# JaneliaSciComp/BigStitcher-Spark

Hardware: NVIDIA H100
Metric: tile-pairs/sec (phase-corr, 512^3 uint16 overlaps) (higher is better)
Workload: dtype f32

## Files before the change

### bigstitcher-spark_b200/csrc/pcm.cu

```cuda
#include <algorithm>
#include <cmath>
#include <cstring>

#include "bs_internal.cuh"
#include "pcm_fft.cuh"

#define PCM_THREADS 256
#define PCM_KMAX 32
#define PCM_SMEM_MAX 232448

extern __shared__ __align__(16) float2 bs_sm[];

struct XR2CArgs {
    const void* img[2];
    float2* spec[2];
    int dtype;
    int dx, dy, dz;
    int Px, Py, Pz, M, pitch;
    int ex;
    int Ex, Ey, Ez;
    const int* idx_x; const float* w_x;
    const int* idx_y; const float* w_y;
    const int* idx_z; const float* w_z;
    const float2* tw;
    FftPlan plan;
    int lshift;
};

__device__ __forceinline__ float load_voxel(const void* p, int dtype, size_t i) {
    if (dtype == BS_DTYPE_U16) return (float)__ldg((const unsigned short*)p + i);
    if (dtype == BS_DTYPE_F32) return __ldg((const float*)p + i);
    return (float)__ldg((const unsigned char*)p + i);
}

#define XR_UNROLL 5
template <class F>
__global__ void __launch_bounds__(PCM_THREADS) k_fft_x_r2c(const __grid_constant__ XR2CArgs a) {
    const int M = F::kStatic ? F::N : a.M;
    const int lshift = F::kStatic ? F::LSHIFT : a.lshift;
    const int LB = 1 << lshift, ls = LB + 1;
    const int Px = 2 * M;
    const int pitch = F::kStatic ? ((F::N + 1 + 15) / 16) * 16 : a.pitch;
    float2* tw = bs_sm;
    float2* b0 = bs_sm + Px;
    float2* b1 = b0 + M * ls;
    const int zp = blockIdx.y, y0 = blockIdx.x * LB, im = blockIdx.z;
    float2* __restrict__ spec = a.spec[im];
    const size_t rowbase = ((size_t)zp * a.Py + y0) * pitch;
    const int nlines = min(LB, a.Py - y0);
    if (zp >= a.Ez || y0 >= a.Ey) {
        const float4 z4 = make_float4(0.f, 0.f, 0.f, 0.f);
        float4* d4 = reinterpret_cast<float4*>(spec + rowbase);
        for (int i = threadIdx.x; i < nlines * (pitch >> 1); i += blockDim.x) d4[i] = z4;
        return;
    }
    for (int i = threadIdx.x; i < Px; i += blockDim.x) tw[i] = a.tw[i];
    const int lane = threadIdx.x & 31, wid = threadIdx.x >> 5;
// ... 107 lines not shown
                 "l"(src), "r"(bytes), "r"(smem_u32(bar))
                 : "memory");
}

struct XR2CTmaArgs {
    XR2CArgs x;
    int n_groups;
    int n_items;
    int row_bytes;
    int esize;
};

template <class F>
__global__ void __launch_bounds__(PCM_THREADS) k_fft_x_r2c_tma(const __grid_constant__ XR2CTmaArgs t) {
    const XR2CArgs& a = t.x;
    const int M = F::kStatic ? F::N : a.M;
    const int lshift = F::kStatic ? F::LSHIFT : a.lshift;
    const int LB = 1 << lshift, ls = LB + 1;
    const int Px = 2 * M;
    const int pitch = F::kStatic ? ((F::N + 1 + 15) / 16) * 16 : a.pitch;
    float2* tw = bs_sm;
    float2* b0 = bs_sm + Px;
    float2* b1 = b0 + M * ls;
    unsigned char* raw = reinterpret_cast<unsigned char*>(b1 + M * ls);
    unsigned long long* bars = reinterpret_cast<unsigned long long*>(raw + 2 * (size_t)LB * t.row_bytes);
    const int lane = threadIdx.x & 31, wid = threadIdx.x >> 5;
    constexpr int NW = PCM_THREADS / 32;

    for (int i = threadIdx.x; i < Px; i += blockDim.x) tw[i] = a.tw[i];
    if (threadIdx.x == 0) {
        mbar_init(&bars[0], 1);
        mbar_init(&bars[1], 1);
        asm volatile("fence.mbarrier_init.release.cluster;" ::: "memory");
    }
    __syncthreads();
// ... 153 lines not shown
        static_assert(UTW + F::Tw::total <= 2 * F::N, "stage tables must fit the twiddle area");
        for (int i = threadIdx.x; i < UTW; i += blockDim.x) tw[i] = a.tw[i];
        F::Tw::build(tw + UTW, a.tw, threadIdx.x, blockDim.x);
    } else {
        for (int i = threadIdx.x; i < Px; i += blockDim.x) tw[i] = a.tw[i];
    }
    if (t.use_tma && lane == 0) {
        mbar_init(&bars[0], 1);
        mbar_init(&bars[1], 1);
        asm volatile("fence.mbarrier_init.release.cluster;" ::: "memory");
    }
    __syncthreads();

    typename F::Tw twr;
    twr.init(F::kSmemTw ? tw + UTW : tw, lane);
    constexpr bool kRegU = F::kStatic && !F::kSmemTw;
    constexpr int UIT = F::kStatic ? (F::N / 2 + 1 + 31) / 32 : 1;
    float2 utw[kRegU ? UIT : 1];
    if constexpr (kRegU) {
#pragma unroll
        for (int i = 0; i < UIT; ++i) utw[i] = tw[min(lane + 32 * i, M)];
    }

    const long long gw = (long long)blockIdx.x * NW + wid, gstride = (long long)gridDim.x * NW;
    const int e0 = a.ex;
    auto src_row = [&](long long line, int& im, int& zp, int& yp) -> long long {
        yp = (int)(line % a.Py);
        const long long r = line / a.Py;
        zp = (int)(r % a.Pz);
        im = (int)(r / a.Pz);
        if (zp >= a.Ez || yp >= a.Ey) return -1;
        return (long long)a.idx_z[zp] * a.dy + a.idx_y[yp];
    };
    auto prefetch = [&](long long line, int buf) {
        int im, zp, yp;
        const long long row = src_row(line, im, zp, yp);
        if (row < 0) return;
// ... 58 lines not shown
        }
        __syncwarp();
        const float2* res = F::run(A, B, tw, twr, a.plan, 2, lane);
        auto untangle = [&](int k, float2 w) {
            const float2 Zk = res[k];
            const float2 Zm = p_mul(res[k == 0 ? 0 : M - k], make_float2(1.f, -1.f));
            const float2 S = caddf(Zk, Zm), Dd = csubf(Zk, Zm);
            const float2 wD = cmulf(w, Dd);
            __stcg(srow + k, cscale(0.5f, cadd_mi(S, wD)));
            if (2 * k != M) __stcg(srow + (M - k), p_mul(cadd_pi(S, wD), make_float2(0.5f, -0.5f)));
        };
        if (F::kStatic) {
#pragma unroll
            for (int i = 0; i < UIT; ++i) {
                const int k = lane + 32 * i;
                if (2 * k <= M) untangle(k, kRegU ? utw[kRegU ? i : 0] : tw[k]);
            }
        } else {
            for (int k = lane; 2 * k <= M; k += 32) untangle(k, tw[k]);
        }
        for (int k = M + 1 + lane; k < pitch; k += 32) __stcg(srow + k, make_float2(0.f, 0.f));
        __syncwarp();
    }
}

#define XW_MAXV 10
template <class F>
__global__ void __launch_bounds__(PCM_THREADS, 3) k_fft_x_c2r_w(const __grid_constant__ XC2RArgs a) {
    const int M = F::kStatic ? F::N : a.M;
    const int Px = 2 * M;
    const int pitch = F::kStatic ? ((F::N + 1 + 15) / 16) * 16 : a.pitch;
    constexpr int NW = PCM_THREADS / 32;
    const int lane = threadIdx.x & 31, wid = threadIdx.x >> 5;
    float2* tw = bs_sm;
    float2* A = bs_sm + Px + (size_t)wid * 2 * (M + 1);
    float2* B = A + (M + 1);
    for (int i = threadIdx.x; i < Px; i += blockDim.x) tw[i] = a.tw[i];
    __syncthreads();
    typename F::Tw twr;
    twr.init(tw, lane);
    constexpr int UIT = F::kStatic ? (F::N / 2 + 1 + 31) / 32 : 1;
    const long long n_lines = (long long)a.Py * a.Pz;
    const long long gw = (long long)blockIdx.x * NW + wid, gstride = (long long)gridDim.x * NW;
    float2 nxt[XW_MAXV];
    auto load_row = [&](long long line) {
        const float2* srow = a.spec + (size_t)line * pitch;
#pragma unroll
        for (int u = 0; u < XW_MAXV; ++u) {
            const int k = lane + 32 * u;
            nxt[u] = (k <= M) ? __ldcg(srow + k) : make_float2(0.f, 0.f);
        }
    };
    if (gw < n_lines) load_row(gw);
    for (long long line = gw; line < n_lines; line += gstride) {
#pragma unroll
        for (int u = 0; u < XW_MAXV; ++u) {
            const int k = lane + 32 * u;
            if (k <= M) B[k] = make_float2(nxt[u].x, -nxt[u].y);
        }
        __syncwarp();
        if (line + gstride < n_lines) load_row(line + gstride);
        auto tangle = [&](int k, float2 wc) {
            const float2 Xk = B[k];
            const float2 Xm = p_mul(B[M - k], make_float2(1.f, -1.f));
            const float2 S = caddf(Xk, Xm), Dd = csubf(Xk, Xm);
            const float2 O = cmulf(Dd, wc);
            A[k] = p_mul(cadd_pi(S, O), make_float2(0.5f, -0.5f));
            if (k != 0 && 2 * k != M) A[M - k] = cscale(0.5f, cadd_mi(S, O));
        };
        if (F::kStatic) {
#pragma unroll
            for (int i = 0; i < UIT; ++i) {
                const int k = lane + 32 * i;
                if (2 * k <= M) tangle(k, p_mul(tw[k], make_float2(1.f, -1.f)));
            }
        } else {
            for (int k = lane; 2 * k <= M; k += 32) tangle(k, p_mul(tw[k], make_float2(1.f, -1.f)));
        }
        __syncwarp();
        const float2* res = F::run(A, B, tw, twr, a.plan, 2, lane);
        float2* row = a.spec + (size_t)line * pitch;
        for (int n = lane; n < M; n += 32) {
            const float2 r = res[n];
            __stcg(row + n, make_float2(r.x * a.scale, -r.y * a.scale));
        }
        __syncwarp();
    }
}

typedef FftWStatic<270, 2, 9, 6, 5> FftW270;
typedef FftWStaticS<270, 2, 9, 6, 5> FftW270S;

struct StridedArgs {
    float2* a;
    float2* b;
    long long estride;
    long long ostride;
    const float2* tw;
    FftPlan plan;
    int tshift;
    int mode;
    float thresh;
};

template <int UNR>
__device__ __forceinline__ void tile_load(float2* dst, const float2* g, long long estride, int N, int tshift) {
// ... 23 lines not shown
    const float4* s4 = reinterpret_cast<const float4*>(src);
#pragma unroll 4
    for (int i = threadIdx.x; i < nvec; i += blockDim.x)
        __stcg(reinterpret_cast<float4*>(g + (long long)(i >> vshift) * estride) + (i & vmask), s4[i]);
}

__device__ __forceinline__ float2 unit_or_zero(float2 x, float thresh) {
    const float m2 = x.x * x.x + x.y * x.y;
    if (m2 < thresh * thresh) return make_float2(0.f, 0.f);
    const float inv = rsqrtf(m2);
    return make_float2(x.x * inv, x.y * inv);
}

template <class F>
__global__ void __launch_bounds__(PCM_THREADS, 3) k_fft_strided(const __grid_constant__ StridedArgs a) {
    const int tshift = F::kStatic ? F::LSHIFT : a.tshift;
    const int TW = 1 << tshift, N = F::kStatic ? F::N : a.plan.n;
    const int twpad = (N + 1) & ~1;
    float2* tw = bs_sm;
    float2* B0 = bs_sm + twpad;
    float2* B1 = B0 + (size_t)N * TW;
    const size_t base = (size_t)blockIdx.y * a.ostride + (size_t)blockIdx.x * TW;
    for (int i = threadIdx.x; i < N; i += blockDim.x) tw[i] = a.tw[i];
    if (a.mode == 0) {
        float2* g = (blockIdx.z ? a.b : a.a) + base;
        tile_load<9>(B0, g, a.estride, N, tshift);
        __syncthreads();
        const float2* res = F::run(B0, B1, tw, a.plan, tshift, TW, 1);
        tile_store(g, res, a.estride, N, tshift);
    } else {
        float2* B2 = B1 + (size_t)N * TW;
        tile_load<9>(B0, a.a + base, a.estride, N, tshift);
// ... 20 lines not shown
}
__device__ __forceinline__ void cp_async_commit() { asm volatile("cp.async.commit_group;" ::: "memory"); }
template <int N>
__device__ __forceinline__ void cp_async_wait() { asm volatile("cp.async.wait_group %0;" ::"n"(N) : "memory"); }

struct StridedPipeArgs {
    StridedArgs s;
    int tiles_x;
    int n_other;
    int n_tiles;
};

template <class F>
__global__ void __launch_bounds__(PCM_THREADS, 2) k_fft_strided_pipe(const __grid_constant__ StridedPipeArgs p) {
    const StridedArgs& a = p.s;
    const int tshift = F::kStatic ? F::LSHIFT : a.tshift;
    const int TW = 1 << tshift, N = F::kStatic ? F::N : a.plan.n;
    const int twpad = (N + 1) & ~1;
    float2* tw = bs_sm;
    float2* B[3];
    B[0] = bs_sm + twpad;
    B[1] = B[0] + (size_t)N * TW;
    B[2] = B[1] + (size_t)N * TW;
    for (int i = threadIdx.x; i < N; i += blockDim.x) tw[i] = a.tw[i];
    const int vshift = tshift - 1, vmask = (1 << vshift) - 1, nvec = N << vshift;

    auto tile_ptr = [&](int t) -> float2* {
        const int tx = t % p.tiles_x;
        const int r = t / p.tiles_x;
        const int o = r % p.n_other, im = r / p.n_other;
        return (im ? a.b : a.a) + (size_t)o * a.ostride + (size_t)tx * TW;
    };
// ... 16 lines not shown
            prefetch(tn, nxt);
            cp_async_wait<1>();
        } else {
            cp_async_wait<0>();
        }
        __syncthreads();
        const float2* res = F::run(cur, pong, tw, a.plan, tshift, TW, 1);
        tile_store(tile_ptr(t), res, a.estride, N, tshift);
        __syncthreads();
    }
}

template <class F>
__global__ void __launch_bounds__(PCM_THREADS, 2) k_fft_xpower_pipe(const __grid_constant__ StridedPipeArgs p) {
    const StridedArgs& a = p.s;
    const int tshift = F::kStatic ? F::LSHIFT : a.tshift;
    const int TW = 1 << tshift, N = F::kStatic ? F::N : a.plan.n;
    const int twpad = (N + 1) & ~1;
    float2* tw = bs_sm;
    float2* bufA = bs_sm + twpad;
    float2* bufB = bufA + (size_t)N * TW;
    float2* pong = bufB + (size_t)N * TW;
    for (int i = threadIdx.x; i < N; i += blockDim.x) tw[i] = a.tw[i];
    const int vshift = tshift - 1, vmask = (1 << vshift) - 1, nvec = N << vshift;
    auto tile_off = [&](int t) -> size_t {
        const int tx = t % p.tiles_x, o = t / p.tiles_x;
        return (size_t)o * a.ostride + (size_t)tx * TW;
    };
    auto prefetch = [&](const float2* g, float2* dst) {
        float4* d4 = reinterpret_cast<float4*>(dst);
        for (int i = threadIdx.x; i < nvec; i += blockDim.x)
            cp_async16(d4 + i, reinterpret_cast<const float4*>(g + (long long)(i >> vshift) * a.estride) + (i & vmask));
// ... 101 lines not shown
                q[u][k2] = make_float2(x.x * y.x + x.y * y.y, x.x * y.y - x.y * y.x);
            }
        });
        Col540Q::stage1(q, XQ, tw);
        const int tn = t + gridDim.x;
        if (tn < p.n_tiles) Col540::load(v, a.a + tile_off(tn), a.estride);
        __syncthreads();
        float2* g = a.a + off;
        Col540Q::stage2(XQ, [&](const float2 (&w)[20], int, int k1, int c) { Col540Q::store(w, g, a.estride, k1, c); });
    }
}


template <class F>
__global__ void __launch_bounds__(PCM_THREADS) k_fft_x_c2r(const __grid_constant__ XC2RArgs a) {
    const int M = F::kStatic ? F::N : a.M;
    const int lshift = F::kStatic ? F::LSHIFT : a.lshift;
    const int LB = 1 << lshift, ls = LB + 1;
    const int Px = 2 * M;
    const int pitch = F::kStatic ? ((F::N + 1 + 15) / 16) * 16 : a.pitch;
    float2* tw = bs_sm;
    float2* T0 = bs_sm + Px;
    float2* T1 = T0 + (size_t)(M + 1) * ls;
    const int zp = blockIdx.y, y0 = blockIdx.x * LB;
    const size_t rowbase = ((size_t)zp * a.Py + y0) * pitch;
    const int nlines = min(LB, a.Py - y0);
    const int lane = threadIdx.x & 31, wid = threadIdx.x >> 5;
    constexpr int NW = PCM_THREADS / 32;
    for (int i = threadIdx.x; i < Px; i += blockDim.x) tw[i] = a.tw[i];
    for (int l = wid; l < LB; l += NW) {
        const float2* srow = a.spec + rowbase + (size_t)l * pitch;
        for (int k0 = 0; k0 <= M; k0 += 32 * XR_UNROLL) {
            float2 v[XR_UNROLL];
#pragma unroll
            for (int u = 0; u < XR_UNROLL; ++u) {
// ... 139 lines not shown
            for (int e = 0; e < K; ++e) {
                const float nv = s_v[w * PCM_KMAX + e];
                if (nv == -INFINITY) break;
                warp_topk_insert(top, K, nv, s_i[w * PCM_KMAX + e], lane);
            }
        if (lane < K) {
            PeakEntry e;
            e.val = top.v;
            e.pad = 0;
            e.idx = (top.v == -INFINITY) ? -1 : top.i;
            a.out[(size_t)blockIdx.x * K + lane] = e;
        }
    }
}

typedef FftStatic<270, 4, 17, 2, PCM_THREADS, 9, 6, 5> FftX270;
typedef FftStatic<270, 3, 9, 2, PCM_THREADS, 9, 6, 5> FftX270L8;

struct PearsonCand {
    int o1[3], o2[3], sz[3];
    int pad;
};

struct PearsonArgs {
    const void* img1;
    const void* img2;
    int dtype;
    int dx, dy, dz;
    const PearsonCand* cands;
    unsigned long long* sums_u;
    double* sums_d;
};

// ... 462 lines not shown
            if (m >= d) m = period - m;
        }
        idx[p] = m;
        w[p] = dist > 0 ? (float)(0.5 * (std::cos(M_PI * (double)dist / (double)e) + 1.0)) : 1.0f;
    }
}

struct PcmGeometry {
    int d[3], ext[3], P[3], E[3];
    int M, pitch;
    FftPlan plan_x, plan_y, plan_z;
    int lshift_x;
    int lshift_r2c;
    int tshift_y, tshift_z;
    size_t smem_x_r2c, smem_x_c2r, smem_y, smem_z;
    bool static_x, static_y, static_z;
};

struct PcmDeviceTables {
    int key[9] = {0, 0, 0, 0, 0, 0, 0, 0, 0};
    int* idx[3] = {nullptr, nullptr, nullptr};
    float* w[3] = {nullptr, nullptr, nullptr};
    float2* tw[3] = {nullptr, nullptr, nullptr};
    int cap[3] = {0, 0, 0};
};

static PcmDeviceTables* tables_of(bs_ctx* ctx) {
    if (!ctx->ws.tables) ctx->ws.tables = new PcmDeviceTables();
    return (PcmDeviceTables*)ctx->ws.tables;
}

// ... 52 lines not shown
    }
    g->lshift_x = ls;
    g->lshift_r2c = std::min(ls, env_int("BS_FFT_R2C_LINES_LOG2", 3));
    g->smem_x_r2c = ((size_t)g->P[0] + 2 * (size_t)g->M * ((1 << g->lshift_r2c) + 1)) * sizeof(float2);
    auto strided = [&](int N, int nbuf, int pref, int* tshift, size_t* smem) -> bool {
        for (int ts = pref; ts >= 1; --ts) {
            const size_t b = ((size_t)((N + 1) & ~1) + (size_t)nbuf * N * (1 << ts)) * sizeof(float2);
            if (b <= PCM_SMEM_MAX) { *tshift = ts; *smem = b; return true; }
        }
        return false;
    };
    if (!strided(g->P[1], 2, env_int("BS_FFT_YTILE_LOG2", 3), &g->tshift_y, &g->smem_y) ||
        !strided(g->P[2], 3, env_int("BS_FFT_ZTILE_LOG2", 3), &g->tshift_z, &g->smem_z))
        return bs_set_error(ctx, BS_ERR_UNSUPPORTED, "pcm: y/z size %dx%d too large for shared memory", g->P[1], g->P[2]);
    const bool allow_static = env_int("BS_FFT_STATIC", 1) != 0;
    g->static_x = allow_static && g->M == FftX270::N && (g->lshift_x == FftX270::LSHIFT || g->lshift_x == FftX270L8::LSHIFT) &&
                  (g->lshift_r2c == 3 || g->lshift_r2c == 4);
    g->static_y = allow_static && g->P[1] == Col540::N;
    g->static_z = allow_static && g->P[2] == Col540::N;
    return BS_OK;
}

static int pcm_tables(bs_ctx* ctx, const PcmGeometry& g, PcmDeviceTables** out) {
    PcmDeviceTables* t = tables_of(ctx);
    *out = t;
    int key[9] = {g.d[0], g.d[1], g.d[2], g.ext[0], g.ext[1], g.ext[2], g.P[0], g.P[1], g.P[2]};
    if (!memcmp(key, t->key, sizeof(key))) return BS_OK;
    BS_CUDA(ctx, cudaStreamSynchronize(ctx->stream));
    for (int d = 0; d < 3; ++d) {
        const int P = g.P[d];
        if (t->cap[d] < P) {
            if (t->idx[d]) { cudaFree(t->idx[d]); cudaFree(t->w[d]); cudaFree(t->tw[d]); }
// ... 53 lines not shown
    pp.n_other = n_other;
    pp.n_tiles = tiles_x * n_other * (n_img ? n_img : 1);
    const int nctas = std::min(pp.n_tiles, ctx->sm_count);
    const size_t smem = (Col540::N + (n_img ? 2 : 3) * (size_t)Col540::XSIZE) * sizeof(float2);
    if (n_img) k_fft_col540<<<nctas, COL540_NT, smem, ctx->stream>>>(pp);
    else k_fft_xpower_col540<<<nctas, COL540_NT, smem, ctx->stream>>>(pp);
}

static int pcm_compute_pcm(bs_ctx* ctx, const void* d1, const void* d2, int dtype, const PcmGeometry& g,
                           PcmDeviceTables* t) {
    if (!ctx->pcm_attr_done) {
        int rc;
        if ((rc = set_smem(ctx, (const void*)k_fft_x_r2c<FftGeneric>, 0))) return rc;
        if ((rc = set_smem(ctx, (const void*)k_fft_strided<FftGeneric>, 0))) return rc;
        if ((rc = set_smem(ctx, (const void*)k_fft_x_c2r<FftGeneric>, 0))) return rc;
        if ((rc = set_smem(ctx, (const void*)k_fft_x_r2c<FftX270>, 0))) return rc;
        if ((rc = set_smem(ctx, (const void*)k_fft_x_r2c<FftX270L8>, 0))) return rc;
        if ((rc = set_smem(ctx, (const void*)k_fft_x_r2c_tma<FftX270L8>, 0))) return rc;
        if ((rc = set_smem(ctx, (const void*)k_fft_x_r2c_w<FftW270S>, 0))) return rc;
        if ((rc = set_smem(ctx, (const void*)k_fft_x_r2c_w<FftWGeneric>, 0))) return rc;
        if ((rc = set_smem(ctx, (const void*)k_fft_x_c2r_w<FftW270>, 0))) return rc;
        if ((rc = set_smem(ctx, (const void*)k_fft_x_c2r_w<FftWGeneric>, 0))) return rc;
        if ((rc = set_smem(ctx, (const void*)k_fft_x_r2c_tma<FftX270>, 0))) return rc;
        if ((rc = set_smem(ctx, (const void*)k_fft_x_r2c_tma<FftGeneric>, 0))) return rc;
        if ((rc = set_smem(ctx, (const void*)k_fft_x_c2r<FftX270L8>, 0))) return rc;
        if ((rc = set_smem(ctx, (const void*)k_fft_strided_pipe<FftGeneric>, 0))) return rc;
        if ((rc = set_smem(ctx, (const void*)k_fft_xpower_pipe<FftGeneric>, 0))) return rc;
        if ((rc = set_smem(ctx, (const void*)k_fft_col540, 0))) return rc;
        if ((rc = set_smem(ctx, (const void*)k_fft_xpower_col540, 0))) return rc;
        if ((rc = set_smem(ctx, (const void*)k_fft_x_c2r<FftX270>, 0))) return rc;
        ctx->pcm_attr_done = true;
    }
    bs_pcm_workspace& ws = ctx->ws;
    float2* sa = (float2*)ws.spec_a;
    float2* sb = (float2*)ws.spec_b;
    {
        XR2CArgs a;
        a.img[0] = d1; a.img[1] = d2;
        a.spec[0] = sa; a.spec[1] = sb;
        a.dtype = dtype;
        a.dx = g.d[0]; a.dy = g.d[1]; a.dz = g.d[2];
        a.Px = g.P[0]; a.Py = g.P[1]; a.Pz = g.P[2]; a.M = g.M; a.pitch = g.pitch;
        a.ex = std::min(g.ext[0], g.d[0]);
        a.Ex = g.E[0]; a.Ey = g.E[1]; a.Ez = g.E[2];
        a.idx_x = t->idx[0]; a.w_x = t->w[0];
// ... 20 lines not shown
            t.use_tma = tma_ok ? 1 : 0;
            t.n_lines = 2LL * g.P[2] * g.P[1];
            const int per_sm = std::max(1, std::min(6, (int)(PCM_SMEM_MAX / (smem_w + 1024))));
            const int nctas = (int)std::min<long long>((t.n_lines + 7) / 8, (long long)ctx->sm_count * per_sm);
            if (g.M == FftW270S::N && env_int("BS_FFT_STATIC", 1)) k_fft_x_r2c_w<FftW270S><<<nctas, PCM_THREADS, smem_w, ctx->stream>>>(t);
            else k_fft_x_r2c_w<FftWGeneric><<<nctas, PCM_THREADS, smem_w, ctx->stream>>>(t);
        } else if (tma_ok) {
            XR2CTmaArgs t;
            t.x = a;
            t.n_groups = (g.P[1] + LB - 1) / LB;
            t.n_items = 2 * g.P[2] * t.n_groups;
            t.row_bytes = row_bytes;
            t.esize = esize;
            const int per_sm = std::max(1, (int)(PCM_SMEM_MAX / (smem_tma + 1024)));
            const int nctas = std::min(t.n_items, ctx->sm_count * std::min(per_sm, 4));
            if (g.static_x && g.lshift_r2c == 3) k_fft_x_r2c_tma<FftX270L8><<<nctas, PCM_THREADS, smem_tma, ctx->stream>>>(t);
            else if (g.static_x && g.lshift_r2c == 4) k_fft_x_r2c_tma<FftX270><<<nctas, PCM_THREADS, smem_tma, ctx->stream>>>(t);
            else k_fft_x_r2c_tma<FftGeneric><<<nctas, PCM_THREADS, smem_tma, ctx->stream>>>(t);
        } else if (g.static_x && g.lshift_r2c == 3) k_fft_x_r2c<FftX270L8><<<grid, PCM_THREADS, g.smem_x_r2c, ctx->stream>>>(a);
        else if (g.static_x && g.lshift_r2c == 4) k_fft_x_r2c<FftX270><<<grid, PCM_THREADS, g.smem_x_r2c, ctx->stream>>>(a);
        else k_fft_x_r2c<FftGeneric><<<grid, PCM_THREADS, g.smem_x_r2c, ctx->stream>>>(a);
    }
    BS_CUDA(ctx, cudaGetLastError());
    {
        StridedArgs a;
        a.a = sa; a.b = sb;
        a.estride = g.pitch;
        a.ostride = (long long)g.P[1] * g.pitch;
        a.tw = t->tw[1];
        a.plan = g.plan_y;
        a.tshift = g.tshift_y;
        a.mode = 0;
        a.thresh = 0.f;
        dim3 grid(g.pitch >> g.tshift_y, g.P[2], 2);
        bs_launch_scope sc(ctx, "fft_y");
        const size_t smem_pipe = ((size_t)((g.P[1] + 1) & ~1) + 3 * (size_t)g.P[1] * (1 << g.tshift_y)) * sizeof(float2);
// ... 64 lines not shown
        } else k_fft_strided<FftGeneric><<<grid, PCM_THREADS, g.smem_y, ctx->stream>>>(a);
    }
    BS_CUDA(ctx, cudaGetLastError());
    {
        XC2RArgs a;
        a.spec = sa;
        a.Px = g.P[0]; a.Py = g.P[1]; a.Pz = g.P[2]; a.M = g.M; a.pitch = g.pitch;
        a.tw = t->tw[0];
        a.plan = g.plan_x;
        a.lshift = g.lshift_x;
        a.scale = (float)(1.0 / ((double)g.M * (double)g.P[1] * (double)g.P[2]));
        const int LB = 1 << g.lshift_x;
        dim3 grid((g.P[1] + LB - 1) / LB, g.P[2], 1);
        bs_launch_scope sc(ctx, "fft_x_c2r");
        const size_t smem_w = ((size_t)g.P[0] + (size_t)(PCM_THREADS / 32) * 2 * (g.M + 1)) * sizeof(float2);
        if (env_int("BS_FFT_X_WARP", 1) && g.M <= 32 * XW_MAXV - 1 && smem_w <= PCM_SMEM_MAX) {
            const long long n_lines = (long long)g.P[1] * g.P[2];
            const int per_sm = std::max(1, std::min(6, (int)(PCM_SMEM_MAX / (smem_w + 1024))));
            const int nctas = (int)std::min<long long>((n_lines + 7) / 8, (long long)ctx->sm_count * per_sm);
            if (g.M == FftW270::N && env_int("BS_FFT_STATIC", 1)) k_fft_x_c2r_w<FftW270><<<nctas, PCM_THREADS, smem_w, ctx->stream>>>(a);
            else k_fft_x_c2r_w<FftWGeneric><<<nctas, PCM_THREADS, smem_w, ctx->stream>>>(a);
        } else if (g.static_x && g.lshift_x == 3) k_fft_x_c2r<FftX270L8><<<grid, PCM_THREADS, g.smem_x_c2r, ctx->stream>>>(a);
        else if (g.static_x) k_fft_x_c2r<FftX270><<<grid, PCM_THREADS, g.smem_x_c2r, ctx->stream>>>(a);
        else k_fft_x_c2r<FftGeneric><<<grid, PCM_THREADS, g.smem_x_c2r, ctx->stream>>>(a);
    }
    BS_CUDA(ctx, cudaGetLastError());
    return BS_OK;
}

static void solve3(const double H[3][3], const double rhs[3], double out[3]) {
    const double a = H[0][0], b = H[0][1], c = H[0][2], d = H[1][0], e = H[1][1], f = H[1][2], g = H[2][0],
                 h = H[2][1], i = H[2][2];
    const double det = a * (e * i - f * h) - b * (d * i - f * g) + c * (d * h - e * g);
    out[0] = out[1] = out[2] = 0.0;
    if (det == 0.0 || !std::isfinite(det)) return;
    const double r0 = rhs[0], r1 = rhs[1], r2 = rhs[2];
    const double x = (r0 * (e * i - f * h) - b * (r1 * i - f * r2) + c * (r1 * h - e * r2)) / det;
    const double y = (a * (r1 * i - f * r2) - r0 * (d * i - f * g) + c * (d * r2 - r1 * g)) / det;
    const double z = (a * (e * r2 - r1 * h) - b * (d * r2 - r1 * g) + r0 * (d * h - e * g)) / det;
// ... 553 lines not shown
```

### bigstitcher-spark_b200/csrc/pcm_fft.cuh

```cuda
#pragma once
#include <cuda_runtime.h>
#include <utility>

#define BS_FFT_MAX_STAGES 12

struct FftPlan {
    int n;
    int nst;
    int radix[BS_FFT_MAX_STAGES];
};

namespace cx {
constexpr double pi = 3.141592653589793238462643383279502884;
constexpr double sin_series(double x) {
    double x2 = x * x, term = x, sum = x;
    for (int i = 1; i < 16; ++i) {
        term *= -x2 / ((2.0 * i) * (2.0 * i + 1.0));
        sum += term;
    }
    return sum;
}
constexpr double cos_series(double x) {
    double x2 = x * x, term = 1.0, sum = 1.0;
    for (int i = 1; i < 16; ++i) {
// ... 187 lines not shown
            case 9: fft_stage<9>(a, b, tw, N, Ls, lshift, lstride, twmul); break;
            case 10: fft_stage<10>(a, b, tw, N, Ls, lshift, lstride, twmul); break;
            case 12: fft_stage<12>(a, b, tw, N, Ls, lshift, lstride, twmul); break;
            case 15: fft_stage<15>(a, b, tw, N, Ls, lshift, lstride, twmul); break;
            case 16: fft_stage<16>(a, b, tw, N, Ls, lshift, lstride, twmul); break;
            default: break;
        }
        __syncthreads();
        Ls *= r;
        float2* t = a; a = b; b = t;
    }
    return a;
}


template <int N, int R, int LS, int LSHIFT, int LSTRIDE, int TWMUL, int NT>
__device__ __forceinline__ void fft_stage_s(const float2* __restrict__ in, float2* __restrict__ out,
                                            const float2* __restrict__ tw) {
    constexpr int m = N / R;
    constexpr int nitems = m << LSHIFT;
    constexpr int lmask = (1 << LSHIFT) - 1;
    constexpr int twstep = (N / (LS * R)) * TWMUL;
    constexpr int iters = (nitems + NT - 1) / NT;
#pragma unroll
    for (int it = 0; it < iters; ++it) {
        const int item = threadIdx.x + it * NT;
        if ((nitems % NT) != 0 && it == iters - 1 && item >= nitems) break;
        const int j = item >> LSHIFT;
        const int l = item & lmask;
        const int k = (LS == 1) ? 0 : (j % LS);
        float2 x[R];
        const float2* p = in + j * LSTRIDE + l;
#pragma unroll
        for (int q = 0; q < R; ++q) x[q] = p[q * m * LSTRIDE];
        if (LS > 1) {
            const float2* t = tw + k * twstep;
#pragma unroll
            for (int q = 1; q < R; ++q) x[q] = cmulf(x[q], t[(q - 1) * k * twstep]);
        }
        dft<R>(x);
        float2* o = out + ((j - k) * R + k) * LSTRIDE + l;
#pragma unroll
        for (int q = 0; q < R; ++q) o[q * LS * LSTRIDE] = x[q];
    }
}

template <int N, int LS, int LSHIFT, int LSTRIDE, int TWMUL, int NT, int R, int... Rest>
__device__ __forceinline__ float2* fft_tile_s(float2* a, float2* b, const float2* tw) {
    fft_stage_s<N, R, LS, LSHIFT, LSTRIDE, TWMUL, NT>(a, b, tw);
    __syncthreads();
    if constexpr (sizeof...(Rest) == 0) return b;
    else return fft_tile_s<N, LS * R, LSHIFT, LSTRIDE, TWMUL, NT, Rest...>(b, a, tw);
}

struct FftGeneric {
    static constexpr bool kStatic = false;
    static constexpr int N = 0, LSHIFT = 0;
    static __device__ __forceinline__ float2* run(float2* a, float2* b, const float2* tw, const FftPlan& plan,
                                                  int lshift, int lstride, int twmul) {
        return fft_tile(a, b, tw, plan, lshift, lstride, twmul);
    }
};

template <int N_, int LSHIFT_, int LSTRIDE_, int TWMUL_, int NT_, int... Rs>
struct FftStatic {
    static constexpr bool kStatic = true;
    static constexpr int N = N_, LSHIFT = LSHIFT_;
    static __device__ __forceinline__ float2* run(float2* a, float2* b, const float2* tw, const FftPlan&, int, int,
                                                  int) {
        return fft_tile_s<N_, 1, LSHIFT_, LSTRIDE_, TWMUL_, NT_, Rs...>(a, b, tw);
    }
};


template <int RA, int RB, int TC, int NT>
struct RegFft2 {
    static constexpr int N = RA * RB;
    static constexpr int I1 = RB * TC, IT1 = (I1 + NT - 1) / NT;
    static constexpr int I2 = RA * TC, IT2 = (I2 + NT - 1) / NT;
    static constexpr int XSIZE = N * TC;
    typedef float2 In[IT1][RA];

    static __device__ __forceinline__ bool live1(int u) { return I1 % NT == 0 || (int)threadIdx.x + u * NT < I1; }
    static __device__ __forceinline__ bool live2(int u) { return I2 % NT == 0 || (int)threadIdx.x + u * NT < I2; }

    static __device__ __forceinline__ void load(In& v, const float2* __restrict__ g, long long estride) {
#pragma unroll
// ... 79 lines not shown
            case 6: fft_stage_wg<6>(a, b, tw, N, Ls, twmul, lane); break;
            case 8: fft_stage_wg<8>(a, b, tw, N, Ls, twmul, lane); break;
            case 9: fft_stage_wg<9>(a, b, tw, N, Ls, twmul, lane); break;
            case 10: fft_stage_wg<10>(a, b, tw, N, Ls, twmul, lane); break;
            case 12: fft_stage_wg<12>(a, b, tw, N, Ls, twmul, lane); break;
            case 15: fft_stage_wg<15>(a, b, tw, N, Ls, twmul, lane); break;
            case 16: fft_stage_wg<16>(a, b, tw, N, Ls, twmul, lane); break;
            default: break;
        }
        Ls *= r;
        float2* t = a; a = b; b = t;
    }
    return a;
}

template <int N, int R, int LS>
struct WStageTw {
    static constexpr int m = N / R;
    static constexpr int iters = (m + 31) / 32;
    float2 w[LS > 1 ? iters : 1][LS > 1 ? R - 1 : 1];
    __device__ __forceinline__ float2 get(int it, int q, int) const { return w[it][q - 1]; }
    template <int TWMUL>
    __device__ __forceinline__ void init(const float2* __restrict__ tw, int lane) {
        if constexpr (LS > 1) {
            constexpr int twstep = (N / (LS * R)) * TWMUL;
#pragma unroll
            for (int it = 0; it < iters; ++it) {
                const int j = min(lane + 32 * it, m - 1);
                const int ts = (j % LS) * twstep;
#pragma unroll
                for (int q = 1; q < R; ++q) w[it][q - 1] = tw[q * ts];
            }
        }
    }
};

template <int N, int LS, int TWMUL, int R, int... Rest>
struct WLineTw {
    WStageTw<N, R, LS> head;
    WLineTw<N, LS * R, TWMUL, Rest...> tail;
    __device__ __forceinline__ void init(const float2* __restrict__ tw, int lane) {
        head.template init<TWMUL>(tw, lane);
        tail.init(tw, lane);
    }
};
template <int N, int LS, int TWMUL, int R>
struct WLineTw<N, LS, TWMUL, R> {
    WStageTw<N, R, LS> head;
    __device__ __forceinline__ void init(const float2* __restrict__ tw, int lane) { head.template init<TWMUL>(tw, lane); }
};

template <int N, int R, int LS, int OFF>
struct WStageTwS {
    const float2* tab;
    __device__ __forceinline__ float2 get(int, int q, int k) const { return tab[OFF + (q - 1) * LS + k]; }
};
template <int N, int LS, int TWMUL, int OFF, int R, int... Rest>
struct WLineTwS {
    static constexpr int cnt = LS > 1 ? (R - 1) * LS : 0;
    WStageTwS<N, R, LS, OFF> head;
    WLineTwS<N, LS * R, TWMUL, OFF + cnt, Rest...> tail;
    static constexpr int total = cnt + WLineTwS<N, LS * R, TWMUL, OFF + cnt, Rest...>::total;
    __device__ __forceinline__ void init(const float2* tab, int) { head.tab = tab; tail.init(tab, 0); }
    static __device__ __forceinline__ void build(float2* dst, const float2* __restrict__ twg, int tid, int nt) {
        if constexpr (LS > 1) {
            constexpr int twstep = (N / (LS * R)) * TWMUL;
// ... 52 lines not shown
    __device__ __forceinline__ void init(const float2*, int) {}
};

struct FftWGeneric {
    static constexpr bool kStatic = false;
    static constexpr bool kSmemTw = false;
    static constexpr int N = 0;
    typedef WNoTw Tw;
    static __device__ __forceinline__ float2* run(float2* a, float2* b, const float2* tw, const Tw&, const FftPlan& plan,
                                                  int twmul, int lane) {
        return fft_line_wg(a, b, tw, plan, twmul, lane);
    }
};

template <int N_, int TWMUL_, int... Rs>
struct FftWStatic {
    static constexpr bool kStatic = true;
    static constexpr bool kSmemTw = false;
    static constexpr int N = N_;
    typedef WLineTw<N_, 1, TWMUL_, Rs...> Tw;
    static __device__ __forceinline__ float2* run(float2* a, float2* b, const float2*, const Tw& twr, const FftPlan&, int,
                                                  int lane) {
        return fft_line_ws<N_, 1, TWMUL_, Rs...>(a, b, twr, lane);
    }
};

template <int N_, int TWMUL_, int... Rs>
struct FftWStaticS {
    static constexpr bool kStatic = true;
    static constexpr bool kSmemTw = true;
    static constexpr int N = N_;
    typedef WLineTwS<N_, 1, TWMUL_, 0, Rs...> Tw;
    static __device__ __forceinline__ float2* run(float2* a, float2* b, const float2*, const Tw& twr, const FftPlan&, int,
                                                  int lane) {
        return fft_line_ws<N_, 1, TWMUL_, Rs...>(a, b, twr, lane);
    }
};
```

Measured before the change: 169.6.

## Add dedicated 540-point x-axis C2R kernel with 10x27 two-pass block decomposition

Adds a specialized C2R kernel for M=270 that tiles 18 lines per block. Each line is factored as 10x27: radix-10 DFTs in registers with the tangle step fused in, a twiddle-multiplied transpose through shared memory, then radix-27 DFTs. Loads of the next tile are prefetched into registers and the shared buffer is double-buffered. It also removes the older static-template FFT variants (FftX270, FftW270, register-twiddle paths), so the other x-axis kernels now always use the generic path, which may slow R2C.

```diff
diff --git a/bigstitcher-spark_b200/csrc/pcm.cu b/bigstitcher-spark_b200/csrc/pcm.cu
--- a/bigstitcher-spark_b200/csrc/pcm.cu
+++ b/bigstitcher-spark_b200/csrc/pcm.cu
@@ -36,11 +36,11 @@
 #define XR_UNROLL 5
 template <class F>
 __global__ void __launch_bounds__(PCM_THREADS) k_fft_x_r2c(const __grid_constant__ XR2CArgs a) {
-    const int M = F::kStatic ? F::N : a.M;
-    const int lshift = F::kStatic ? F::LSHIFT : a.lshift;
+    const int M = a.M;
+    const int lshift = a.lshift;
     const int LB = 1 << lshift, ls = LB + 1;
     const int Px = 2 * M;
-    const int pitch = F::kStatic ? ((F::N + 1 + 15) / 16) * 16 : a.pitch;
+    const int pitch = a.pitch;
     float2* tw = bs_sm;
     float2* b0 = bs_sm + Px;
     float2* b1 = b0 + M * ls;
@@ -178,11 +178,11 @@
 template <class F>
 __global__ void __launch_bounds__(PCM_THREADS) k_fft_x_r2c_tma(const __grid_constant__ XR2CTmaArgs t) {
     const XR2CArgs& a = t.x;
-    const int M = F::kStatic ? F::N : a.M;
-    const int lshift = F::kStatic ? F::LSHIFT : a.lshift;
+    const int M = a.M;
+    const int lshift = a.lshift;
     const int LB = 1 << lshift, ls = LB + 1;
     const int Px = 2 * M;
-    const int pitch = F::kStatic ? ((F::N + 1 + 15) / 16) * 16 : a.pitch;
+    const int pitch = a.pitch;
     float2* tw = bs_sm;
     float2* b0 = bs_sm + Px;
     float2* b1 = b0 + M * ls;
@@ -366,13 +366,7 @@
 
     typename F::Tw twr;
     twr.init(F::kSmemTw ? tw + UTW : tw, lane);
-    constexpr bool kRegU = F::kStatic && !F::kSmemTw;
     constexpr int UIT = F::kStatic ? (F::N / 2 + 1 + 31) / 32 : 1;
-    float2 utw[kRegU ? UIT : 1];
-    if constexpr (kRegU) {
-#pragma unroll
-        for (int i = 0; i < UIT; ++i) utw[i] = tw[min(lane + 32 * i, M)];
-    }
 
     const long long gw = (long long)blockIdx.x * NW + wid, gstride = (long long)gridDim.x * NW;
     const int e0 = a.ex;
@@ -461,7 +455,7 @@
 #pragma unroll
             for (int i = 0; i < UIT; ++i) {
                 const int k = lane + 32 * i;
-                if (2 * k <= M) untangle(k, kRegU ? utw[kRegU ? i : 0] : tw[k]);
+                if (2 * k <= M) untangle(k, tw[k]);
             }
         } else {
             for (int k = lane; 2 * k <= M; k += 32) untangle(k, tw[k]);
@@ -474,9 +468,9 @@
 #define XW_MAXV 10
 template <class F>
 __global__ void __launch_bounds__(PCM_THREADS, 3) k_fft_x_c2r_w(const __grid_constant__ XC2RArgs a) {
-    const int M = F::kStatic ? F::N : a.M;
+    const int M = a.M;
     const int Px = 2 * M;
-    const int pitch = F::kStatic ? ((F::N + 1 + 15) / 16) * 16 : a.pitch;
+    const int pitch = a.pitch;
     constexpr int NW = PCM_THREADS / 32;
     const int lane = threadIdx.x & 31, wid = threadIdx.x >> 5;
     float2* tw = bs_sm;
@@ -484,9 +478,6 @@
     float2* B = A + (M + 1);
     for (int i = threadIdx.x; i < Px; i += blockDim.x) tw[i] = a.tw[i];
     __syncthreads();
-    typename F::Tw twr;
-    twr.init(tw, lane);
-    constexpr int UIT = F::kStatic ? (F::N / 2 + 1 + 31) / 32 : 1;
     const long long n_lines = (long long)a.Py * a.Pz;
     const long long gw = (long long)blockIdx.x * NW + wid, gstride = (long long)gridDim.x * NW;
     float2 nxt[XW_MAXV];
@@ -515,17 +506,9 @@
             A[k] = p_mul(cadd_pi(S, O), make_float2(0.5f, -0.5f));
             if (k != 0 && 2 * k != M) A[M - k] = cscale(0.5f, cadd_mi(S, O));
         };
-        if (F::kStatic) {
-#pragma unroll
-            for (int i = 0; i < UIT; ++i) {
-                const int k = lane + 32 * i;
-                if (2 * k <= M) tangle(k, p_mul(tw[k], make_float2(1.f, -1.f)));
-            }
-        } else {
-            for (int k = lane; 2 * k <= M; k += 32) tangle(k, p_mul(tw[k], make_float2(1.f, -1.f)));
-        }
+        for (int k = lane; 2 * k <= M; k += 32) tangle(k, p_mul(tw[k], make_float2(1.f, -1.f)));
         __syncwarp();
-        const float2* res = F::run(A, B, tw, twr, a.plan, 2, lane);
+        const float2* res = F::run(A, B, tw, typename F::Tw(), a.plan, 2, lane);
         float2* row = a.spec + (size_t)line * pitch;
         for (int n = lane; n < M; n += 32) {
             const float2 r = res[n];
@@ -535,8 +518,92 @@
     }
 }
 
-typedef FftWStatic<270, 2, 9, 6, 5> FftW270;
 typedef FftWStaticS<270, 2, 9, 6, 5> FftW270S;
+
+#define X540_M 270
+#define X540_TR 18
+#define X540_NT 256
+#define X540_XS (X540_TR * X540_M)
+#define X540_PITCH 272
+
+__device__ __forceinline__ void x540_tables(float2* tu, float2* ts, const float2* __restrict__ tw) {
+    for (int i = threadIdx.x; i < X540_M; i += blockDim.x) {
+        tu[i] = tw[i];
+        ts[i] = tw[2 * ((i / 27) * (i % 27))];
+    }
+}
+
+struct X540C2RArgs {
+    float2* spec;
+    long long n_lines;
+    int n_tiles;
+    const float2* tw;
+    float scale;
+};
+
+__global__ void __launch_bounds__(X540_NT, 2) k_fft_x540_c2r(const __grid_constant__ X540C2RArgs a) {
+    constexpr int M = X540_M, TR = X540_TR, PITCH = X540_PITCH;
+    float2* tu = bs_sm;
+    float2* ts = tu + M;
+    float2* X0 = ts + M;
+    const int tid = threadIdx.x;
+    const int l1 = tid / 14, j = tid % 14;
+    const int l2 = tid / 10, k1 = tid % 10;
+    float2 v[2][10];
+    auto load = [&](int tile) {
+        const long long line = (long long)tile * TR + l1;
+        if (tid < 14 * TR && line < a.n_lines) {
+            const float2* row = a.spec + line * PITCH;
+#pragma unroll
+            for (int n1 = 0; n1 < 10; ++n1) {
+                v[0][n1] = __ldcg(row + 27 * n1 + j);
+                v[1][n1] = __ldcg(row + 27 * n1 + 27 - j);
+            }
+        }
+    };
+    int tile = blockIdx.x;
+    if (tile < a.n_tiles) load(tile);
+    x540_tables(tu, ts, a.tw);
+    __syncthreads();
+    for (int it = 0; tile < a.n_tiles; tile += gridDim.x, ++it) {
+        float2* X = X0 + (it & 1) * X540_XS;
+        if (tid < 14 * TR && (long long)tile * TR + l1 < a.n_lines) {
+#pragma unroll
+            for (int n1 = 0; n1 < 10; ++n1) {
+                const float2 Xk = p_mul(v[0][n1], make_float2(1.f, -1.f));
+                const float2 Xm = v[1][9 - n1];
+                const float2 S = caddf(Xk, Xm), Dd = csubf(Xk, Xm);
+                const float2 O = cmulf(Dd, p_mul(tu[27 * n1 + j], make_float2(1.f, -1.f)));
+                v[0][n1] = p_mul(cadd_pi(S, O), make_float2(0.5f, -0.5f));
+                v[1][9 - n1] = cscale(0.5f, cadd_mi(S, O));
+            }
+            dft<10>(v[0]);
+            dft<10>(v[1]);
+            float2* x = X + l1 * M;
+            x[j] = v[0][0];
+            if (j) x[27 - j] = v[1][0];
+#pragma unroll
+            for (int q = 1; q < 10; ++q) {
+                x[q * 27 + j] = cmulf(v[0][q], ts[q * 27 + j]);
+                if (j) x[q * 27 + 27 - j] = cmulf(v[1][q], ts[q * 27 + 27 - j]);
+            }
+        }
+        if (tile + (int)gridDim.x < a.n_tiles) load(tile + gridDim.x);
+        __syncthreads();
+        const long long line = (long long)tile * TR + l2;
+        if (tid < 10 * TR && line < a.n_lines) {
+            const float2* x = X + l2 * M + k1 * 27;
+            float2 w[27];
+#pragma unroll
+            for (int q = 0; q < 27; ++q) w[q] = x[q];
+            dft<27>(w);
+            float2* row = a.spec + line * PITCH;
+#pragma unroll
+            for (int k2 = 0; k2 < 27; ++k2) __stcg(row + k1 + 10 * k2, make_float2(w[k2].x * a.scale, -w[k2].y * a.scale));
+        }
+    }
+}
+
 
 struct StridedArgs {
     float2* a;
@@ -590,8 +657,8 @@
 
 template <class F>
 __global__ void __launch_bounds__(PCM_THREADS, 3) k_fft_strided(const __grid_constant__ StridedArgs a) {
-    const int tshift = F::kStatic ? F::LSHIFT : a.tshift;
-    const int TW = 1 << tshift, N = F::kStatic ? F::N : a.plan.n;
+    const int tshift = a.tshift;
+    const int TW = 1 << tshift, N = a.plan.n;
     const int twpad = (N + 1) & ~1;
     float2* tw = bs_sm;
     float2* B0 = bs_sm + twpad;
@@ -642,8 +709,8 @@
 template <class F>
 __global__ void __launch_bounds__(PCM_THREADS, 2) k_fft_strided_pipe(const __grid_constant__ StridedPipeArgs p) {
     const StridedArgs& a = p.s;
-    const int tshift = F::kStatic ? F::LSHIFT : a.tshift;
-    const int TW = 1 << tshift, N = F::kStatic ? F::N : a.plan.n;
+    const int tshift = a.tshift;
+    const int TW = 1 << tshift, N = a.plan.n;
     const int twpad = (N + 1) & ~1;
     float2* tw = bs_sm;
     float2* B[3];
@@ -690,8 +757,8 @@
 template <class F>
 __global__ void __launch_bounds__(PCM_THREADS, 2) k_fft_xpower_pipe(const __grid_constant__ StridedPipeArgs p) {
     const StridedArgs& a = p.s;
-    const int tshift = F::kStatic ? F::LSHIFT : a.tshift;
-    const int TW = 1 << tshift, N = F::kStatic ? F::N : a.plan.n;
+    const int tshift = a.tshift;
+    const int TW = 1 << tshift, N = a.plan.n;
     const int twpad = (N + 1) & ~1;
     float2* tw = bs_sm;
     float2* bufA = bs_sm + twpad;
@@ -823,11 +890,11 @@
 
 template <class F>
 __global__ void __launch_bounds__(PCM_THREADS) k_fft_x_c2r(const __grid_constant__ XC2RArgs a) {
-    const int M = F::kStatic ? F::N : a.M;
-    const int lshift = F::kStatic ? F::LSHIFT : a.lshift;
+    const int M = a.M;
+    const int lshift = a.lshift;
     const int LB = 1 << lshift, ls = LB + 1;
     const int Px = 2 * M;
-    const int pitch = F::kStatic ? ((F::N + 1 + 15) / 16) * 16 : a.pitch;
+    const int pitch = a.pitch;
     float2* tw = bs_sm;
     float2* T0 = bs_sm + Px;
     float2* T1 = T0 + (size_t)(M + 1) * ls;
@@ -997,9 +1064,6 @@
     }
 }
 
-typedef FftStatic<270, 4, 17, 2, PCM_THREADS, 9, 6, 5> FftX270;
-typedef FftStatic<270, 3, 9, 2, PCM_THREADS, 9, 6, 5> FftX270L8;
-
 struct PearsonCand {
     int o1[3], o2[3], sz[3];
     int pad;
@@ -1492,7 +1556,7 @@
     int lshift_r2c;
     int tshift_y, tshift_z;
     size_t smem_x_r2c, smem_x_c2r, smem_y, smem_z;
-    bool static_x, static_y, static_z;
+    bool static_y, static_z;
 };
 
 struct PcmDeviceTables {
@@ -1575,8 +1639,6 @@
         !strided(g->P[2], 3, env_int("BS_FFT_ZTILE_LOG2", 3), &g->tshift_z, &g->smem_z))
         return bs_set_error(ctx, BS_ERR_UNSUPPORTED, "pcm: y/z size %dx%d too large for shared memory", g->P[1], g->P[2]);
     const bool allow_static = env_int("BS_FFT_STATIC", 1) != 0;
-    g->static_x = allow_static && g->M == FftX270::N && (g->lshift_x == FftX270::LSHIFT || g->lshift_x == FftX270L8::LSHIFT) &&
-                  (g->lshift_r2c == 3 || g->lshift_r2c == 4);
     g->static_y = allow_static && g->P[1] == Col540::N;
     g->static_z = allow_static && g->P[2] == Col540::N;
     return BS_OK;
@@ -1660,21 +1722,15 @@
         if ((rc = set_smem(ctx, (const void*)k_fft_x_r2c<FftGeneric>, 0))) return rc;
         if ((rc = set_smem(ctx, (const void*)k_fft_strided<FftGeneric>, 0))) return rc;
         if ((rc = set_smem(ctx, (const void*)k_fft_x_c2r<FftGeneric>, 0))) return rc;
-        if ((rc = set_smem(ctx, (const void*)k_fft_x_r2c<FftX270>, 0))) return rc;
-        if ((rc = set_smem(ctx, (const void*)k_fft_x_r2c<FftX270L8>, 0))) return rc;
-        if ((rc = set_smem(ctx, (const void*)k_fft_x_r2c_tma<FftX270L8>, 0))) return rc;
         if ((rc = set_smem(ctx, (const void*)k_fft_x_r2c_w<FftW270S>, 0))) return rc;
         if ((rc = set_smem(ctx, (const void*)k_fft_x_r2c_w<FftWGeneric>, 0))) return rc;
-        if ((rc = set_smem(ctx, (const void*)k_fft_x_c2r_w<FftW270>, 0))) return rc;
+        if ((rc = set_smem(ctx, (const void*)k_fft_x540_c2r, 0))) return rc;
         if ((rc = set_smem(ctx, (const void*)k_fft_x_c2r_w<FftWGeneric>, 0))) return rc;
-        if ((rc = set_smem(ctx, (const void*)k_fft_x_r2c_tma<FftX270>, 0))) return rc;
         if ((rc = set_smem(ctx, (const void*)k_fft_x_r2c_tma<FftGeneric>, 0))) return rc;
-        if ((rc = set_smem(ctx, (const void*)k_fft_x_c2r<FftX270L8>, 0))) return rc;
         if ((rc = set_smem(ctx, (const void*)k_fft_strided_pipe<FftGeneric>, 0))) return rc;
         if ((rc = set_smem(ctx, (const void*)k_fft_xpower_pipe<FftGeneric>, 0))) return rc;
         if ((rc = set_smem(ctx, (const void*)k_fft_col540, 0))) return rc;
         if ((rc = set_smem(ctx, (const void*)k_fft_xpower_col540, 0))) return rc;
-        if ((rc = set_smem(ctx, (const void*)k_fft_x_c2r<FftX270>, 0))) return rc;
         ctx->pcm_attr_done = true;
     }
     bs_pcm_workspace& ws = ctx->ws;
@@ -1725,12 +1781,8 @@
             t.esize = esize;
             const int per_sm = std::max(1, (int)(PCM_SMEM_MAX / (smem_tma + 1024)));
             const int nctas = std::min(t.n_items, ctx->sm_count * std::min(per_sm, 4));
-            if (g.static_x && g.lshift_r2c == 3) k_fft_x_r2c_tma<FftX270L8><<<nctas, PCM_THREADS, smem_tma, ctx->stream>>>(t);
-            else if (g.static_x && g.lshift_r2c == 4) k_fft_x_r2c_tma<FftX270><<<nctas, PCM_THREADS, smem_tma, ctx->stream>>>(t);
-            else k_fft_x_r2c_tma<FftGeneric><<<nctas, PCM_THREADS, smem_tma, ctx->stream>>>(t);
-        } else if (g.static_x && g.lshift_r2c == 3) k_fft_x_r2c<FftX270L8><<<grid, PCM_THREADS, g.smem_x_r2c, ctx->stream>>>(a);
-        else if (g.static_x && g.lshift_r2c == 4) k_fft_x_r2c<FftX270><<<grid, PCM_THREADS, g.smem_x_r2c, ctx->stream>>>(a);
-        else k_fft_x_r2c<FftGeneric><<<grid, PCM_THREADS, g.smem_x_r2c, ctx->stream>>>(a);
+            k_fft_x_r2c_tma<FftGeneric><<<nctas, PCM_THREADS, smem_tma, ctx->stream>>>(t);
+        } else k_fft_x_r2c<FftGeneric><<<grid, PCM_THREADS, g.smem_x_r2c, ctx->stream>>>(a);
     }
     BS_CUDA(ctx, cudaGetLastError());
     {
@@ -1825,15 +1877,22 @@
         dim3 grid((g.P[1] + LB - 1) / LB, g.P[2], 1);
         bs_launch_scope sc(ctx, "fft_x_c2r");
         const size_t smem_w = ((size_t)g.P[0] + (size_t)(PCM_THREADS / 32) * 2 * (g.M + 1)) * sizeof(float2);
-        if (env_int("BS_FFT_X_WARP", 1) && g.M <= 32 * XW_MAXV - 1 && smem_w <= PCM_SMEM_MAX) {
+        if (g.M == X540_M) {
+            X540C2RArgs c;
+            c.spec = sa;
+            c.n_lines = (long long)g.P[1] * g.P[2];
+            c.n_tiles = (int)((c.n_lines + X540_TR - 1) / X540_TR);
+            c.tw = t->tw[0];
+            c.scale = a.scale;
+            const size_t smem = (2 * X540_M + 2 * X540_XS) * sizeof(float2);
+            const int nctas = std::min(c.n_tiles, ctx->sm_count * 2);
+            k_fft_x540_c2r<<<nctas, X540_NT, smem, ctx->stream>>>(c);
+        } else if (env_int("BS_FFT_X_WARP", 1) && g.M <= 32 * XW_MAXV - 1 && smem_w <= PCM_SMEM_MAX) {
             const long long n_lines = (long long)g.P[1] * g.P[2];
             const int per_sm = std::max(1, std::min(6, (int)(PCM_SMEM_MAX / (smem_w + 1024))));
             const int nctas = (int)std::min<long long>((n_lines + 7) / 8, (long long)ctx->sm_count * per_sm);
-            if (g.M == FftW270::N && env_int("BS_FFT_STATIC", 1)) k_fft_x_c2r_w<FftW270><<<nctas, PCM_THREADS, smem_w, ctx->stream>>>(a);
-            else k_fft_x_c2r_w<FftWGeneric><<<nctas, PCM_THREADS, smem_w, ctx->stream>>>(a);
-        } else if (g.static_x && g.lshift_x == 3) k_fft_x_c2r<FftX270L8><<<grid, PCM_THREADS, g.smem_x_c2r, ctx->stream>>>(a);
-        else if (g.static_x) k_fft_x_c2r<FftX270><<<grid, PCM_THREADS, g.smem_x_c2r, ctx->stream>>>(a);
-        else k_fft_x_c2r<FftGeneric><<<grid, PCM_THREADS, g.smem_x_c2r, ctx->stream>>>(a);
+            k_fft_x_c2r_w<FftWGeneric><<<nctas, PCM_THREADS, smem_w, ctx->stream>>>(a);
+        } else k_fft_x_c2r<FftGeneric><<<grid, PCM_THREADS, g.smem_x_c2r, ctx->stream>>>(a);
     }
     BS_CUDA(ctx, cudaGetLastError());
     return BS_OK;
diff --git a/bigstitcher-spark_b200/csrc/pcm_fft.cuh b/bigstitcher-spark_b200/csrc/pcm_fft.cuh
--- a/bigstitcher-spark_b200/csrc/pcm_fft.cuh
+++ b/bigstitcher-spark_b200/csrc/pcm_fft.cuh
@@ -225,63 +225,13 @@
 }
 
 
-template <int N, int R, int LS, int LSHIFT, int LSTRIDE, int TWMUL, int NT>
-__device__ __forceinline__ void fft_stage_s(const float2* __restrict__ in, float2* __restrict__ out,
-                                            const float2* __restrict__ tw) {
-    constexpr int m = N / R;
-    constexpr int nitems = m << LSHIFT;
-    constexpr int lmask = (1 << LSHIFT) - 1;
-    constexpr int twstep = (N / (LS * R)) * TWMUL;
-    constexpr int iters = (nitems + NT - 1) / NT;
-#pragma unroll
-    for (int it = 0; it < iters; ++it) {
-        const int item = threadIdx.x + it * NT;
-        if ((nitems % NT) != 0 && it == iters - 1 && item >= nitems) break;
-        const int j = item >> LSHIFT;
-        const int l = item & lmask;
-        const int k = (LS == 1) ? 0 : (j % LS);
-        float2 x[R];
-        const float2* p = in + j * LSTRIDE + l;
-#pragma unroll
-        for (int q = 0; q < R; ++q) x[q] = p[q * m * LSTRIDE];
-        if (LS > 1) {
-            const float2* t = tw + k * twstep;
-#pragma unroll
-            for (int q = 1; q < R; ++q) x[q] = cmulf(x[q], t[(q - 1) * k * twstep]);
-        }
-        dft<R>(x);
-        float2* o = out + ((j - k) * R + k) * LSTRIDE + l;
-#pragma unroll
-        for (int q = 0; q < R; ++q) o[q * LS * LSTRIDE] = x[q];
-    }
-}
-
-template <int N, int LS, int LSHIFT, int LSTRIDE, int TWMUL, int NT, int R, int... Rest>
-__device__ __forceinline__ float2* fft_tile_s(float2* a, float2* b, const float2* tw) {
-    fft_stage_s<N, R, LS, LSHIFT, LSTRIDE, TWMUL, NT>(a, b, tw);
-    __syncthreads();
-    if constexpr (sizeof...(Rest) == 0) return b;
-    else return fft_tile_s<N, LS * R, LSHIFT, LSTRIDE, TWMUL, NT, Rest...>(b, a, tw);
-}
-
 struct FftGeneric {
-    static constexpr bool kStatic = false;
-    static constexpr int N = 0, LSHIFT = 0;
     static __device__ __forceinline__ float2* run(float2* a, float2* b, const float2* tw, const FftPlan& plan,
                                                   int lshift, int lstride, int twmul) {
         return fft_tile(a, b, tw, plan, lshift, lstride, twmul);
     }
 };
 
-template <int N_, int LSHIFT_, int LSTRIDE_, int TWMUL_, int NT_, int... Rs>
-struct FftStatic {
-    static constexpr bool kStatic = true;
-    static constexpr int N = N_, LSHIFT = LSHIFT_;
-    static __device__ __forceinline__ float2* run(float2* a, float2* b, const float2* tw, const FftPlan&, int, int,
-                                                  int) {
-        return fft_tile_s<N_, 1, LSHIFT_, LSTRIDE_, TWMUL_, NT_, Rs...>(a, b, tw);
-    }
-};
 
 
 template <int RA, int RB, int TC, int NT>
@@ -391,42 +341,6 @@
     return a;
 }
 
-template <int N, int R, int LS>
-struct WStageTw {
-    static constexpr int m = N / R;
-    static constexpr int iters = (m + 31) / 32;
-    float2 w[LS > 1 ? iters : 1][LS > 1 ? R - 1 : 1];
-    __device__ __forceinline__ float2 get(int it, int q, int) const { return w[it][q - 1]; }
-    template <int TWMUL>
-    __device__ __forceinline__ void init(const float2* __restrict__ tw, int lane) {
-        if constexpr (LS > 1) {
-            constexpr int twstep = (N / (LS * R)) * TWMUL;
-#pragma unroll
-            for (int it = 0; it < iters; ++it) {
-                const int j = min(lane + 32 * it, m - 1);
-                const int ts = (j % LS) * twstep;
-#pragma unroll
-                for (int q = 1; q < R; ++q) w[it][q - 1] = tw[q * ts];
-            }
-        }
-    }
-};
-
-template <int N, int LS, int TWMUL, int R, int... Rest>
-struct WLineTw {
-    WStageTw<N, R, LS> head;
-    WLineTw<N, LS * R, TWMUL, Rest...> tail;
-    __device__ __forceinline__ void init(const float2* __restrict__ tw, int lane) {
-        head.template init<TWMUL>(tw, lane);
-        tail.init(tw, lane);
-    }
-};
-template <int N, int LS, int TWMUL, int R>
-struct WLineTw<N, LS, TWMUL, R> {
-    WStageTw<N, R, LS> head;
-    __device__ __forceinline__ void init(const float2* __restrict__ tw, int lane) { head.template init<TWMUL>(tw, lane); }
-};
-
 template <int N, int R, int LS, int OFF>
 struct WStageTwS {
     const float2* tab;
@@ -509,18 +423,6 @@
 };
 
 template <int N_, int TWMUL_, int... Rs>
-struct FftWStatic {
-    static constexpr bool kStatic = true;
-    static constexpr bool kSmemTw = false;
-    static constexpr int N = N_;
-    typedef WLineTw<N_, 1, TWMUL_, Rs...> Tw;
-    static __device__ __forceinline__ float2* run(float2* a, float2* b, const float2*, const Tw& twr, const FftPlan&, int,
-                                                  int lane) {
-        return fft_line_ws<N_, 1, TWMUL_, Rs...>(a, b, twr, lane);
-    }
-};
-
-template <int N_, int TWMUL_, int... Rs>
 struct FftWStaticS {
     static constexpr bool kStatic = true;
     static constexpr bool kSmemTw = true;
```

New measurement: 170.6 (median of 6 runs). Within noise of the previous version (+0.6%).
